# yuhang1008/WildGS-SLAM-Blackwell

Hardware: AMD Instinct MI355X
Metric: rasterised Gaussians/s fwd+bwd @1M pts 1080p; PSNR vs ref (higher is better)
Workload: dtype f32; 1 GPU; configs[2]: 1000000 Gaussians, 1920x1080, SH3, single-view fwd+bwd, pose grad on; gaussians=1000000, image=1920x1080, sh_degree=3, num_rendered=13015374, parallelism=dp1 (keyframe views), dp_exchange=none

## Files before the change

### wildgs-slam-blackwell_amd/csrc/capi.hip

```cpp
#include <cstdarg>
#include <cstdio>
#include <cstdlib>
#include <cstring>
#include <vector>

#include <immintrin.h>

#include "wgsr.h"
#include "wgsr_common.h"
#include "wgsr_internal.h"

namespace wgsr {

namespace {
thread_local char g_err[1024] = "";

struct HostCounters {
  uint32_t* buf = nullptr;
  hipEvent_t ev = nullptr;
  hipStream_t side = nullptr;
  hipEvent_t pre = nullptr;
  uint4* mbox = nullptr;
  uint32_t seq = 0;
};
// ... 109 lines not shown
        ms[r.stage] += t;
        count[r.stage] += 1;
      }
      pool.push_back(r.a);
      pool.push_back(r.b);
    }
    recs.clear();
  }
};
Prof g_prof;

struct StageTimer {
  Stage stage;
  hipStream_t s;
  hipEvent_t a = nullptr;
  StageTimer(Stage st, hipStream_t str) : stage(st), s(str) {
    if (((g_prof.mask >> st) & 1u) && (a = g_prof.get()) && hipEventRecord(a, s) != hipSuccess) a = nullptr;
  }
  ~StageTimer() {
    if (!a) return;
    hipEvent_t b = g_prof.get();
    if (b && hipEventRecord(b, s) == hipSuccess) g_prof.recs.push_back({stage, a, b});
    else g_prof.pool.push_back(a);
  }
};

struct Grid {
  int gx, gy, nt;
  explicit Grid(const wgsr_raster_args& a)
      : gx((a.W + kTile - 1) / kTile), gy((a.H + kTile - 1) / kTile), nt(gx * gy) {}
};

int sort_bits(int n) { return num_bits((uint32_t)n) > 0 ? num_bits((uint32_t)n) : 1; }

constexpr int kDefaultBinShift = 2;
constexpr int kSmallFrameTiles = 2048;
int bin_shift(const wgsr_raster_args& a) {
  const char* e = getenv("WGSR_BIN_SHIFT");
  const Grid g(a);
  int sh = e ? atoi(e) : (g.nt <= kSmallFrameTiles ? 1 : kDefaultBinShift);
  sh = sh < 0 ? 0 : (sh > kMaxBinShift ? kMaxBinShift : sh);
  return sh > 0 && g.nt > 65535 ? 0 : sh;
}
enum class DepthSched { kBins, kGlobal, kFull };
DepthSched depth_schedule(int bshift) {
  const char* e = getenv("WGSR_DEPTH_SORT");
  if (e && strcmp(e, "full") == 0) return DepthSched::kFull;
  if (!bshift || (e && strcmp(e, "global") == 0)) return DepthSched::kGlobal;
  return DepthSched::kBins;
}
size_t bin_depth_max_avg() {
  const char* e = getenv("WGSR_BIN_DEPTH_MAX_AVG");
  return e ? (size_t)strtoull(e, nullptr, 10) : (size_t)6144;
}
constexpr int kDepthBits = 32;
constexpr bool kFullDepthInAlt = ((kDepthBits + 7) / 8) % 2 == 1;
thread_local int64_t g_depth_order_off = -1;

int validate(const wgsr_raster_args* a) {
  if (!a) return set_error(WGSR_EINVAL, "null args");
  if (a->P < 0) return set_error(WGSR_EINVAL, "means3D must have dimensions (num_points, 3)");
  if (a->W <= 0 || a->H <= 0) return set_error(WGSR_EINVAL, "image size must be positive (got %dx%d)", a->W, a->H);
  if (a->P == 0) return WGSR_OK;
  if (!a->means3D || !a->opacities || !a->bg || !a->viewmatrix || !a->projmatrix || !a->campos)
    return set_error(WGSR_EINVAL, "missing required tensor");
  if ((a->shs == nullptr) == (a->colors == nullptr))
    return set_error(WGSR_EINVAL, "Please provide excatly one of either SHs or precomputed colors!");
  const bool sr = a->scales && a->rotations;
  if (sr == (a->cov3D_precomp != nullptr))
    return set_error(WGSR_EINVAL,
                     "Please provide exactly one of either scale/rotation pair or precomputed 3D covariance!");
  if (a->shs && (a->M <= 0 || a->D < 0 || a->D > 3 || (a->D + 1) * (a->D + 1) > a->M))
    return set_error(WGSR_EINVAL, "invalid SH configuration (degree %d, %d coefficients)", a->D, a->M);
  const Grid g(*a);
  if (g.gx > 65535 || g.gy > 65535) return set_error(WGSR_EINVAL, "image too large");
  return WGSR_OK;
}

#define HIPCHK(expr)                                                                          \
  do {                                                                                        \
    hipError_t _e = (expr);                                                                   \
    if (_e != hipSuccess) return set_error(WGSR_EHIP, "%s: %s", #expr, hipGetErrorString(_e)); \
  } while (0)

#define STAGE(a, s, expr)                   \
  do {                                      \
    HIPCHK(expr);                           \
    if ((a).debug) {                        \
      HIPCHK(hipStreamSynchronize(s));      \
      HIPCHK(hipGetLastError());            \
    }                                       \
  } while (0)

void* call_alloc(wgsr_alloc_fn fn, void* ctx, size_t bytes) { return fn ? fn(ctx, bytes) : nullptr; }

struct Fwd {
  const wgsr_raster_args& a;
  hipStream_t s;
  Grid grid; GeomLayout GL; ImageLayout IL;
  int bshift;
  float *out_color, *out_depth, *out_opacity;
  int32_t* n_touched;
  void *geom = nullptr, *image = nullptr;
  uint32_t* counter = nullptr;
  template <typename T> T* g(size_t off) const { return at<T>(geom, off); }
  template <typename T> T* im(size_t off) const { return at<T>(image, off); }
// ... 153 lines not shown
}

int queue_depth_fixup(const Fwd& f, HostCounters& hc, const Counts& c, const uint32_t** depth_order) {
  const GeomLayout& GL = f.GL;
  uint32_t hi = 0, nlo = 0;
  if (int e = read_depth_range(f, hc, c, &hi, &nlo)) return e;
  const DepthKeyPlan pl = depth_key_plan(hi, ~nlo);
  if (pl.extra_bits <= 0) return WGSR_OK;
  bool alt = false;
  { StageTimer T(kStDepthSort, f.s);
  STAGE(f.a, f.s, radix_sort_pairs(f.g<uint32_t>(GL.dkey_alt), f.g<uint32_t>(GL.dkey), f.g<uint32_t>(GL.dval_alt),
                                   f.g<uint32_t>(GL.dval), false, (size_t)f.a.P, pl.extra_shift, pl.R,
                                   f.g<uint32_t>(GL.hist), f.g<uint32_t>(GL.totals), f.s, &alt)); }
  *depth_order = f.g<uint32_t>(alt ? GL.dval : GL.dval_alt);
  return requeue_scan(f, *depth_order);
}

int queue_lists_and_render(const Fwd& f, void* binning, const BinningPlan& plan, const uint32_t* depth_order,
                           bool bin_depth, size_t NL, const uint32_t* ndev) {
  const wgsr_raster_args& a = f.a;
  hipStream_t s = f.s;
  const int bshift = f.bshift;
  const BinLayout& BL = plan.BL;
  uint32_t* lists = at<uint32_t>(binning, bshift ? BL.total : BL.point_g);
  uint2 *ranges = f.im<uint2>(f.IL.ranges), *tile_m = f.im<uint2>(f.IL.tile_m);
  uint32_t *tile_len = f.im<uint32_t>(f.IL.tile_len), *meta = f.im<uint32_t>(f.IL.meta);
  const uint32_t *sorted_keys = nullptr, *sorted_gid = nullptr;
  bool emit = false, bounds_done = false;
  if (NL > 0) {
    const int bits = sort_bits(bshift ? Bins(f.grid.gx, f.grid.gy, bshift).n : f.grid.nt);
    const bool odd = radix_passes(0, bits) % 2 == 1;
    uint32_t* vin = at<uint32_t>(binning, odd ? BL.slot_g : BL.point_g);
    uint32_t* valt = at<uint32_t>(binning, odd ? BL.point_g : BL.slot_g);
    size_t bs_off = 0;
    const size_t bs_words = bshift ? sort_sup_words(NL, 0, bits, &bs_off) : 0;
    ZeroJob zb{};
    zb.p[0] = reinterpret_cast<float*>(at<uint32_t>(binning, BL.hist) + bs_off);
    zb.n[0] = bs_words;
    zb.count = bs_words ? 1 : 0;
    { StageTimer T(kStDuplicate, s);
    if (bshift) {
      const uint32_t cap = ndev ? (uint32_t)NL : 0xFFFFFFFFu;
      STAGE(a, s, launch_duplicate_bins(a, f.geom, depth_order, bshift, at<uint8_t>(binning, BL.flag),
                                        at<uint32_t>(binning, BL.key), vin, true, zb, meta, s, cap, cap));
    } else {
      STAGE(a, s, launch_duplicate(a, f.geom, depth_order, (uint32_t)a.P, at<uint32_t>(binning, BL.key), vin,
                                   at<uint8_t>(binning, BL.flag), s));
    } }
    bool talt = false;
    uint2* bin_bounds = (bshift && (size_t)8 << bits <= (size_t)16 * f.grid.nt) ? tile_m : nullptr;
    { StageTimer T(kStTileSort, s);
    STAGE(a, s, radix_sort_pairs(at<uint32_t>(binning, BL.key), at<uint32_t>(binning, BL.key_alt), vin, valt, false,
                                 NL, 0, bits, at<uint32_t>(binning, BL.hist), at<uint32_t>(binning, BL.totals), s,
                                 &talt, bin_bounds, &bounds_done, bs_words != 0, ndev)); }
    if (talt != odd) return set_error(WGSR_EHIP, "internal: list sort parity");
    if (ndev && !bounds_done) return set_error(WGSR_EHIP, "internal: capacity mode without the sort's bin bounds");
    sorted_keys = at<uint32_t>(binning, talt ? BL.key_alt : BL.key);
    sorted_gid = at<uint32_t>(binning, BL.point_g);
    emit = bin_depth && bds_emit(bshift);
    if (bin_depth) {
      StageTimer T(kStTileSort, s);
      uint32_t* okeys = at<uint32_t>(binning, talt ? BL.key : BL.key_alt);
      uint32_t* ogid = at<uint32_t>(binning, BL.slot_g);
      STAGE(a, s, launch_bin_depth_sort(a, sorted_keys, sorted_gid, (uint32_t)NL, bshift, tile_m, bounds_done,
                                        at<uint32_t>(f.geom, f.GL.dkey), okeys, ogid,
                                        at<char>(binning, BL.total + plan.lists_bytes), s, emit ? lists : nullptr,
                                        ranges, tile_len, meta));
      bounds_done = true;
      if (!emit) {
        sorted_keys = okeys;
        sorted_gid = ogid;
      }
    }
  }
  { StageTimer T(kStRanges, s);
  if (emit) {
  } else if (bshift && NL > 0) {
    STAGE(a, s, launch_expand_bins(a, sorted_keys, sorted_gid, (uint32_t)NL, bshift, tile_m, bounds_done, lists,
                                   ranges, tile_len, meta, s));
  } else {
    STAGE(a, s, launch_ranges(sorted_keys, (uint32_t)NL, f.grid.nt, ranges, tile_len, meta, s));
  } }
  StageTimer T(kStRenderFwd, s);
  STAGE(a, s, launch_render_fwd(a, ranges, lists, f.geom, f.out_color, f.out_depth, f.out_opacity,
                                f.im<float>(f.IL.final_T), f.im<uint32_t>(f.IL.n_contrib), f.n_touched,
                                f.im<uint32_t>(f.IL.tile_m), s));
  return WGSR_OK;
}

}
}

using namespace wgsr;

extern "C" {

const char* wgsr_last_error(void) { return g_err; }

void wgsr_profile_enable(int on) {
  g_prof.flush();
  g_prof.mask = on == 1 ? ((1u << WGSR_NUM_STAGES) - 1u) : (on > 1 ? ((uint32_t)on >> 1) : 0u);
}

int wgsr_profile_read(double* ms, int64_t* counts, int n, int reset) {
  g_prof.flush();
  const int m = n < WGSR_NUM_STAGES ? n : WGSR_NUM_STAGES;
  for (int i = 0; i < m; ++i) {
// ... 333 lines not shown
```

### wildgs-slam-blackwell_amd/csrc/sort.hip

```cpp
#include <stdlib.h>
#include <string.h>

#include "wgsr_common.h"
#include "wgsr_internal.h"

namespace wgsr {

namespace {

__device__ __forceinline__ uint32_t block_excl_scan256(uint32_t v, uint32_t* s_tmp4, uint32_t* total) {
  const int t = threadIdx.x, w = t >> 6, lane = t & 63;
  uint32_t inc = wave_incl_scan(v);
  if (lane == 63) s_tmp4[w] = inc;
  __syncthreads();
  uint32_t base = 0, tot = 0;
#pragma unroll
  for (int i = 0; i < 4; ++i) {
    uint32_t x = s_tmp4[i];
    base += (i < w) ? x : 0u;
    tot += x;
  }
  __syncthreads();
  if (total) *total = tot;
  return base + inc - v;
}


template <int I>
__device__ __forceinline__ int load_run(const uint32_t* __restrict__ keys, size_t n, size_t e0, uint32_t (&k)[I]) {
  static_assert(I % 4 == 0, "load_run reads uint4s");
  if (e0 + I <= n) {
    const uint4* p = reinterpret_cast<const uint4*>(keys + e0);
#pragma unroll
    for (int q = 0; q < I / 4; ++q) {
      const uint4 v = p[q];
      k[4 * q] = v.x; k[4 * q + 1] = v.y; k[4 * q + 2] = v.z; k[4 * q + 3] = v.w;
    }
    return I;
  }
  const int nv = e0 < n ? (int)(n - e0) : 0;
#pragma unroll
  for (int j = 0; j < I; ++j) k[j] = j < nv ? keys[e0 + j] : 0u;
  return nv;
}

template <int I>
__device__ __forceinline__ void add_runs(uint32_t* h, const uint32_t (&k)[I], int nv, int shift, uint32_t mask) {
  if (nv <= 0) return;
  uint32_t cur = (k[0] >> shift) & mask, run = 0;
#pragma unroll
  for (int j = 0; j < I; ++j) {
    if (j < nv) {
      const uint32_t d = (k[j] >> shift) & mask;
      if (d != cur) {
        atomicAdd(&h[cur], run);
        cur = d;
        run = 0;
      }
      ++run;
    }
  }
  atomicAdd(&h[cur], run);
}

constexpr uint32_t kSupBlocks = kSortSupBlocks;
template <int I>
__global__ __launch_bounds__(256) void k_radix_hist(const uint32_t* __restrict__ keys, uint32_t n, int shift,
                                                    int bits, uint32_t nb, uint32_t* __restrict__ hist,
                                                    uint32_t* __restrict__ sup, uint32_t nsup,
                                                    const uint32_t* __restrict__ ndev) {
  __shared__ uint32_t s_h[256];
  const int t = threadIdx.x;
  if (ndev) n = min(n, *ndev);
  s_h[t] = 0;
  uint32_t k[I];
  const int nv = load_run<I>(keys, n, (size_t)blockIdx.x * (256 * I) + (size_t)t * I, k);
  __syncthreads();
  add_runs(s_h, k, nv, shift, (1u << bits) - 1u);
  __syncthreads();
  const uint32_t c = s_h[t];
  if (sup) {
    hist[(size_t)blockIdx.x * 256 + t] = c;
    if (c) atomicAdd(&sup[(size_t)(blockIdx.x / kSupBlocks) * 256 + t], c);
  } else {
// ... 86 lines not shown
  uint32_t gdig = 0;
  if (sup) {
    gdig = sup_digit_base(hist, sup, nb, nsup, bid, t, s_tmp, bounds, mask);
  } else {
    const uint32_t ex = block_excl_scan256(totals[t], s_tmp, nullptr);
    gdig = ex + hist[(size_t)t * nb + bid];
  }
#pragma unroll
  for (int j = 0; j < I; ++j) {
    const size_t e = base + (size_t)j * 64 + lane;
    const bool valid = e < n;
    const uint32_t d = (key[j] >> shift) & mask;
    const uint64_t peers = match_digit(d, bits, wave_ballot(valid));
    const int leader = __ffsll((unsigned long long)peers) - 1;
    uint32_t old = 0;
    if (valid && lane == leader) old = atomicAdd(&s_wcnt[w][d], (uint32_t)__popcll(peers));
    old = (uint32_t)__shfl((int)old, leader & 63, 64);
    rank[j] = old + lanes_below(peers);
  }
  __syncthreads();
  {
    const uint32_t c0 = s_wcnt[0][t], c1 = s_wcnt[1][t], c2 = s_wcnt[2][t], c3 = s_wcnt[3][t];
    const uint32_t cnt_d = c0 + c1 + c2 + c3;
    s_wcnt[0][t] = 0;
    s_wcnt[1][t] = c0;
    s_wcnt[2][t] = c0 + c1;
    s_wcnt[3][t] = c0 + c1 + c2;
    s_lbase[t] = block_excl_scan256(cnt_d, s_tmp, nullptr);
    s_gbase[t] = gdig;
  }
  __syncthreads();
#pragma unroll
  for (int j = 0; j < I; ++j) {
    const size_t e = base + (size_t)j * 64 + lane;
    const uint32_t d = (key[j] >> shift) & mask;
    const uint32_t slot = s_lbase[d] + s_wcnt[w][d] + rank[j];
    if (e < n) s_buf[slot] = make_uint2(key[j], val[j]);
  }
  __syncthreads();
  const uint32_t cnt = (size_t)n > blk0 ? (uint32_t)min((size_t)kTile, (size_t)n - blk0) : 0u;
#pragma unroll
  for (int r = 0; r < I; ++r) {
    const uint32_t i = (uint32_t)t + 256u * r;
    if (i < cnt) {
      const uint2 kv = s_buf[i];
      const uint32_t d = (kv.x >> shift) & mask;
      const uint32_t dst = s_gbase[d] + (i - s_lbase[d]);
      kout[dst] = kv.x;
      vout[dst] = kv.y;
    }
  }
}

template <int DIG, int I>
__global__ __launch_bounds__(256) void k_radix_hist_wide(const uint32_t* __restrict__ keys, uint32_t n, int shift,
                                                         int bits, uint32_t nb, uint32_t* __restrict__ hist,
                                                         const uint32_t* __restrict__ ndev) {
  __shared__ uint32_t s_h[DIG];
  const int t = threadIdx.x;
  if (ndev) n = min(n, *ndev);
#pragma unroll
  for (int k = 0; k < DIG / 256; ++k) s_h[t + 256 * k] = 0;
  uint32_t key[I];
  const int nv = load_run<I>(keys, n, (size_t)blockIdx.x * (256 * I) + (size_t)t * I, key);
  __syncthreads();
  add_runs(s_h, key, nv, shift, (1u << bits) - 1u);
  __syncthreads();
#pragma unroll
  for (int k = 0; k < DIG / 256; ++k) hist[(size_t)(t + 256 * k) * nb + blockIdx.x] = s_h[t + 256 * k];
}

template <int DIG, int I>
__global__ __launch_bounds__(256) void k_radix_scatter_wide(
    const uint32_t* __restrict__ kin, const uint32_t* __restrict__ vin, int iota, uint32_t n, int shift, int bits,
    uint32_t nb, const uint32_t* __restrict__ hist, const uint32_t* __restrict__ totals, uint32_t* __restrict__ kout,
    uint32_t* __restrict__ vout, uint2* __restrict__ digit_bounds, const uint32_t* __restrict__ ndev) {
  constexpr int kT = 256 * I, DPT = DIG / 256;
  if (ndev) {
    n = min(n, *ndev);
    if ((size_t)blockIdx.x * kT >= n && !(blockIdx.x == 0 && digit_bounds)) return;
  }
  __shared__ uint2 s_buf[kT];
  __shared__ uint32_t s_wcnt[4][DIG];
  __shared__ uint32_t s_lbase[DIG];
  __shared__ uint32_t s_gbase[DIG];
  __shared__ uint32_t s_tmp[4];
  const int t = threadIdx.x, w = t >> 6, lane = t & 63;
  const uint32_t mask = (1u << bits) - 1u;
#pragma unroll
  for (int i = 0; i < 4 * DPT; ++i) (&s_wcnt[0][0])[t + 256 * i] = 0;
  const uint32_t bid = blockIdx.x;
  const size_t blk0 = (size_t)bid * kT;
  const size_t base = blk0 + (size_t)w * (64 * I);
  uint32_t key[I], val[I], rank[I];
#pragma unroll
  for (int j = 0; j < I; ++j) {
    const size_t e = base + (size_t)j * 64 + lane;
    const bool valid = e < n;
    key[j] = valid ? kin[e] : 0u;
    val[j] = iota ? (uint32_t)e : (valid ? vin[e] : 0u);
  }
  {
    uint32_t tot[DPT], s = 0;
#pragma unroll
    for (int k = 0; k < DPT; ++k) { tot[k] = totals[t * DPT + k]; s += tot[k]; }
    uint32_t run = block_excl_scan256(s, s_tmp, nullptr);
#pragma unroll
    for (int k = 0; k < DPT; ++k) {
      const int d = t * DPT + k;
      s_gbase[d] = run + hist[(size_t)d * nb + bid];
      if (digit_bounds && bid == 0) digit_bounds[d] = make_uint2(run, run + tot[k]);
      run += tot[k];
    }
  }
#pragma unroll
  for (int j = 0; j < I; ++j) {
    const size_t e = base + (size_t)j * 64 + lane;
    const bool valid = e < n;
    const uint32_t d = (key[j] >> shift) & mask;
    const uint64_t peers = match_digit(d, bits, wave_ballot(valid));
    const int leader = __ffsll((unsigned long long)peers) - 1;
    uint32_t old = 0;
    if (valid && lane == leader) old = atomicAdd(&s_wcnt[w][d], (uint32_t)__popcll(peers));
    old = (uint32_t)__shfl((int)old, leader & 63, 64);
    rank[j] = old + lanes_below(peers);
  }
  __syncthreads();
  {
    uint32_t cnt[DPT], s = 0;
#pragma unroll
    for (int k = 0; k < DPT; ++k) {
      const int d = t * DPT + k;
      const uint32_t c0 = s_wcnt[0][d], c1 = s_wcnt[1][d], c2 = s_wcnt[2][d], c3 = s_wcnt[3][d];
      cnt[k] = c0 + c1 + c2 + c3;
      s += cnt[k];
      s_wcnt[0][d] = 0;
      s_wcnt[1][d] = c0;
      s_wcnt[2][d] = c0 + c1;
      s_wcnt[3][d] = c0 + c1 + c2;
    }
    uint32_t run = block_excl_scan256(s, s_tmp, nullptr);
#pragma unroll
    for (int k = 0; k < DPT; ++k) {
      s_lbase[t * DPT + k] = run;
      run += cnt[k];
    }
  }
  __syncthreads();
#pragma unroll
  for (int j = 0; j < I; ++j) {
    const size_t e = base + (size_t)j * 64 + lane;
    const uint32_t d = (key[j] >> shift) & mask;
    const uint32_t slot = s_lbase[d] + s_wcnt[w][d] + rank[j];
    if (e < n) s_buf[slot] = make_uint2(key[j], val[j]);
  }
  __syncthreads();
  const uint32_t cnt = (size_t)n > blk0 ? (uint32_t)min((size_t)kT, (size_t)n - blk0) : 0u;
#pragma unroll
  for (int r = 0; r < I; ++r) {
    const uint32_t i = (uint32_t)t + 256u * r;
    if (i < cnt) {
      const uint2 kv = s_buf[i];
      const uint32_t d = (kv.x >> shift) & mask;
      const uint32_t dst = s_gbase[d] + (i - s_lbase[d]);
      kout[dst] = kv.x;
      vout[dst] = kv.y;
    }
  }
}

static_assert(kRectPairLanes == 64, "one range word per lane");
__device__ __forceinline__ int bitlen32(uint32_t x) {
  return x ? 32 - __clz((int)x) : 0;
}
__device__ __forceinline__ uint32_t wave_max_u32_uniform(uint32_t x) {
  x = max(x, (uint32_t)__builtin_amdgcn_update_dpp(0, (int)x, 0xB1, 0xf, 0xf, true));
  x = max(x, (uint32_t)__builtin_amdgcn_update_dpp(0, (int)x, 0x4E, 0xf, 0xf, true));
  x = max(x, (uint32_t)__builtin_amdgcn_update_dpp(0, (int)x, 0x114, 0xf, 0xf, true));
  x = max(x, (uint32_t)__builtin_amdgcn_update_dpp(0, (int)x, 0x118, 0xf, 0xf, true));
  const uint32_t a = (uint32_t)__builtin_amdgcn_readlane((int)x, 15), b = (uint32_t)__builtin_amdgcn_readlane((int)x, 31);
  const uint32_t c = (uint32_t)__builtin_amdgcn_readlane((int)x, 47), d = (uint32_t)__builtin_amdgcn_readlane((int)x, 63);
  return max(max(a, b), max(c, d));
}
__device__ __forceinline__ uint2 depth_range_reduce(const uint32_t* __restrict__ range) {
  const int lane = threadIdx.x & 63;
  return make_uint2(wave_max_u32_uniform(range[lane]), wave_max_u32_uniform(range[kRectPairLanes + lane]));
}
__device__ __forceinline__ DepthKeyPlan depth_plan_from2(const uint32_t* __restrict__ range2) {
  return depth_key_plan(range2[0], ~range2[1]);
}

template <int I, int PASS>
__global__ __launch_bounds__(256) void k_depth_hist(const uint32_t* __restrict__ keys, uint32_t n,
                                                    const uint32_t* __restrict__ range, uint32_t* __restrict__ range2,
                                                    uint32_t* __restrict__ hist, uint32_t* __restrict__ sup) {
  __shared__ uint32_t s_h[kDepthMaxDigits];
  const int t = threadIdx.x;
  uint32_t k[I];
  const int nv = load_run<I>(keys, n, (size_t)blockIdx.x * (256 * I) + (size_t)t * I, k);
#pragma unroll
  for (int q = 0; q < kDepthMaxDigits / 256; ++q) s_h[t + 256 * q] = 0;
  DepthKeyPlan pl;
  if (PASS == 0) {
    const uint2 r = depth_range_reduce(range);
    if (blockIdx.x == 0 && t == 0) {
      range2[0] = r.x;
      range2[1] = r.y;
    }
    pl = depth_key_plan(r.x, ~r.y);
  } else {
    pl = depth_plan_from2(range2);
  }
  const int shift = pl.shift[PASS], bits = pl.bits[PASS];
// ... 269 lines not shown
  const uint32_t b0 = min(nbs, t * per), b1 = min(nbs, b0 + per);
  uint2 acc = make_uint2(0u, 0u);
  for (uint32_t b = b0; b < b1; b += 8) {
    uint2 v[8];
#pragma unroll
    for (int u = 0; u < 8; ++u) v[u] = b + u < b1 ? bsum[b + u] : make_uint2(0u, 0u);
#pragma unroll
    for (int u = 0; u < 8; ++u) { acc.x += v[u].x; acc.y += v[u].y; }
  }
  const uint32_t ia = wave_incl_scan(acc.x), ib = wave_incl_scan(acc.y);
  if (lane == 63) s_w[w] = make_uint2(ia, ib);
  __syncthreads();
  uint2 run = make_uint2(ia - acc.x, ib - acc.y), tot = make_uint2(0u, 0u);
#pragma unroll
  for (int k = 0; k < NW; ++k) {
    const uint2 x = s_w[k];
    if (k < w) { run.x += x.x; run.y += x.y; }
    tot.x += x.x;
    tot.y += x.y;
  }
  for (uint32_t b = b0; b < b1; b += 8) {
    uint2 v[8];
#pragma unroll
    for (int u = 0; u < 8; ++u) v[u] = b + u < b1 ? bsum[b + u] : make_uint2(0u, 0u);
#pragma unroll
    for (int u = 0; u < 8; ++u) {
      if (b + u < b1) bsum[b + u] = run;
      run.x += v[u].x;
      run.y += v[u].y;
    }
  }
  if (t == 0) bsum[nbs] = tot;
}

}

static bool wide_pass(int bits) { return bits > 8 && bits <= 10; }

int radix_passes(int begin_bit, int end_bit) {
  const int bits = end_bit - begin_bit;
  if (bits <= 0) return 0;
  return wide_pass(bits) ? 1 : (bits + 7) / 8;
}

size_t sort_sup_words(size_t n, int begin_bit, int end_bit, size_t* offset_words) {
  const int bits = end_bit - begin_bit;
  if (offset_words) *offset_words = 0;
  if (n == 0 || bits <= 0 || wide_pass(bits)) return 0;
  const uint32_t nb = sort_blocks(n);
  if (offset_words) *offset_words = 256 * (size_t)nb;
  return 256 * (size_t)((nb + kSupBlocks - 1) / kSupBlocks) * ((bits + 7) / 8);
}

template <int I>
static hipError_t radix_sort_tiled(uint32_t* keys, uint32_t* keys_alt, uint32_t* vals, uint32_t* vals_alt,
                                   bool vals_iota, size_t n, int begin_bit, int end_bit, uint32_t* status,
                                   uint32_t* totals, hipStream_t stream, bool* result_in_alt, uint2* digit_bounds,
                                   bool* bounds_done, bool sup_zeroed, const uint32_t* ndev) {
  const uint32_t nb = sort_blocks(n);
  if (wide_pass(end_bit - begin_bit) && n <= (size_t)kStCount) {
    const int bits = end_bit - begin_bit;
    if (bits <= 9) {
      hipLaunchKernelGGL((k_radix_hist_wide<512, I>), dim3(nb), dim3(256), 0, stream, keys, (uint32_t)n, begin_bit,
                         bits, nb, status, ndev);
      hipLaunchKernelGGL(k_radix_rowscan, dim3(512), dim3(256), 0, stream, status, nb, totals);
      hipLaunchKernelGGL((k_radix_scatter_wide<512, I>), dim3(nb), dim3(256), 0, stream, keys, vals,
                         vals_iota ? 1 : 0, (uint32_t)n, begin_bit, bits, nb, status, totals, keys_alt, vals_alt,
                         begin_bit == 0 ? digit_bounds : nullptr, ndev);
    } else {
      hipLaunchKernelGGL((k_radix_hist_wide<1024, I>), dim3(nb), dim3(256), 0, stream, keys, (uint32_t)n, begin_bit,
                         bits, nb, status, ndev);
      hipLaunchKernelGGL(k_radix_rowscan, dim3(1024), dim3(256), 0, stream, status, nb, totals);
      hipLaunchKernelGGL((k_radix_scatter_wide<1024, I>), dim3(nb), dim3(256), 0, stream, keys, vals,
                         vals_iota ? 1 : 0, (uint32_t)n, begin_bit, bits, nb, status, totals, keys_alt, vals_alt,
                         begin_bit == 0 ? digit_bounds : nullptr, ndev);
    }
    *result_in_alt = true;
    if (bounds_done) *bounds_done = digit_bounds && begin_bit == 0;
    return hipGetLastError();
  }
  const int passes = (end_bit - begin_bit + 7) / 8;
  if (passes > kMaxSortPasses || n > (size_t)kStCount) return hipErrorInvalidValue;
  uint32_t* ghist = totals;
  const uint32_t nsup = (nb + kSupBlocks - 1) / kSupBlocks;
  uint32_t* sup = status + 256 * (size_t)nb;
  if (!sup_zeroed) {
    hipError_t e = hipMemsetAsync(sup, 0, 4 * 256 * (size_t)nsup * passes, stream);
    if (e != hipSuccess) return e;
  }
  uint32_t *ki = keys, *ko = keys_alt, *vi = vals, *vo = vals_alt;
  bool iota = vals_iota;
  const int per = (end_bit - begin_bit + passes - 1) / passes;
  for (int p = 0; p < passes; ++p) {
    const int shift = begin_bit + per * p;
    const int bits = min(per, end_bit - shift);
    uint32_t* sp = sup + (size_t)p * 256 * nsup;
    hipLaunchKernelGGL(k_radix_hist<I>, dim3(nb), dim3(256), 0, stream, ki, (uint32_t)n, shift, bits, nb, status,
                       sp, nsup, ndev);
    uint2* db = (passes == 1 && begin_bit == 0) ? digit_bounds : nullptr;
    hipLaunchKernelGGL(k_radix_scatter<I>, dim3(nb), dim3(256), 0, stream, ki, vi, iota ? 1 : 0, (uint32_t)n, shift,
                       bits, nb, status, ghist, ko, vo, sp, nsup, db, ndev);
    if (db && bounds_done) *bounds_done = true;
    iota = false;
    uint32_t* tk = ki; ki = ko; ko = tk;
    uint32_t* tv = vi; vi = vo; vo = tv;
    *result_in_alt = !*result_in_alt;
  }
  return hipGetLastError();
}

hipError_t radix_sort_pairs(uint32_t* keys, uint32_t* keys_alt, uint32_t* vals, uint32_t* vals_alt, bool vals_iota,
                            size_t n, int begin_bit, int end_bit, uint32_t* status, uint32_t* totals,
                            hipStream_t stream, bool* result_in_alt, uint2* digit_bounds, bool* bounds_done,
                            bool sup_zeroed, const uint32_t* ndev) {
  *result_in_alt = false;
  if (bounds_done) *bounds_done = false;
  if (n == 0 || end_bit <= begin_bit) {
    if (vals_iota && n > 0) {
      return hipErrorInvalidValue;
    }
    return hipSuccess;
  }
  switch (sort_items(n)) {
    case kTinySortItems:
      return radix_sort_tiled<kTinySortItems>(keys, keys_alt, vals, vals_alt, vals_iota, n, begin_bit, end_bit, status,
                                              totals, stream, result_in_alt, digit_bounds, bounds_done, sup_zeroed,
                                              ndev);
    case kSmallSortItems:
      return radix_sort_tiled<kSmallSortItems>(keys, keys_alt, vals, vals_alt, vals_iota, n, begin_bit, end_bit,
                                               status, totals, stream, result_in_alt, digit_bounds, bounds_done,
                                               sup_zeroed, ndev);
    default:
      return radix_sort_tiled<kSortItems>(keys, keys_alt, vals, vals_alt, vals_iota, n, begin_bit, end_bit, status,
                                          totals, stream, result_in_alt, digit_bounds, bounds_done, sup_zeroed,
                                          ndev);
  }
}

template <int I>
static hipError_t depth_sort_tiled(uint32_t* keys, uint32_t* keys_alt, uint32_t* vals, uint32_t* vals_alt, size_t n,
                                   const uint32_t* range, uint32_t* range2, uint32_t* scratch, hipStream_t s) {
  const uint32_t nb = (uint32_t)((n + 256 * I - 1) / (256 * I)), nsup = (nb + kSupBlocks - 1) / kSupBlocks;
  uint32_t* hist = scratch;
  uint32_t* sup = scratch + depth_sort_sup_offset_words(n);
  const size_t sup_pass = (size_t)kDepthMaxDigits * nsup;
  const uint32_t un = (uint32_t)n;
  hipLaunchKernelGGL((k_depth_hist<I, 0>), dim3(nb), dim3(256), 0, s, keys, un, range, range2, hist, sup);
  hipLaunchKernelGGL((k_depth_scatter<I, 0>), dim3(nb), dim3(256), 0, s, keys, vals, un, range2, hist, sup, nsup,
                     keys_alt, vals_alt);
  hipLaunchKernelGGL((k_depth_hist<I, 1>), dim3(nb), dim3(256), 0, s, keys_alt, un, range, range2, hist,
                     sup + sup_pass);
  hipLaunchKernelGGL((k_depth_scatter<I, 1>), dim3(nb), dim3(256), 0, s, keys_alt, vals_alt, un, range2, hist,
                     sup + sup_pass, nsup, keys, vals);
  hipLaunchKernelGGL((k_depth_hist<I, 2>), dim3(nb), dim3(256), 0, s, keys, un, range, range2, hist,
                     sup + 2 * sup_pass);
  hipLaunchKernelGGL((k_depth_scatter<I, 2>), dim3(nb), dim3(256), 0, s, keys, vals, un, range2, hist,
                     sup + 2 * sup_pass, nsup, keys_alt, vals_alt);
  return hipGetLastError();
}

hipError_t launch_depth_sort(uint32_t* keys, uint32_t* keys_alt, uint32_t* vals, uint32_t* vals_alt, size_t n,
                             const uint32_t* range, uint32_t* range2, uint32_t* scratch, hipStream_t s) {
  if (n == 0) return hipSuccess;
  if (n > (size_t)kStCount) return hipErrorInvalidValue;
  switch (sort_items(n)) {
    case kTinySortItems:
      return depth_sort_tiled<kTinySortItems>(keys, keys_alt, vals, vals_alt, n, range, range2, scratch, s);
    case kSmallSortItems:
      return depth_sort_tiled<kSmallSortItems>(keys, keys_alt, vals, vals_alt, n, range, range2, scratch, s);
    default:
      return depth_sort_tiled<kSortItems>(keys, keys_alt, vals, vals_alt, n, range, range2, scratch, s);
  }
}

hipError_t exclusive_scan_gather(const uint32_t* vals, const uint32_t* idx, size_t n, uint32_t* out,
                                 uint32_t* scatter_out, uint32_t* bsum, uint32_t* total_out, hipStream_t stream,
                                 uint32_t stride) {
  const uint32_t nbs = (uint32_t)((n + kScanTile - 1) / kScanTile);
  if (n == 0) {
    hipError_t e = hipMemsetAsync(out, 0, sizeof(uint32_t), stream);
    if (e == hipSuccess && total_out) e = hipMemsetAsync(total_out, 0, sizeof(uint32_t), stream);
    return e;
  }
  hipLaunchKernelGGL(k_scan_reduce, dim3(nbs), dim3(256), 0, stream, vals, stride, idx, (uint32_t)n, bsum);
  hipLaunchKernelGGL(k_scan_bsum, dim3(1), dim3(256), 0, stream, bsum, nbs, total_out);
  hipLaunchKernelGGL(k_scan_down, dim3(nbs), dim3(256), 0, stream, vals, stride, idx, (uint32_t)n, bsum, out,
                     scatter_out);
  return hipGetLastError();
// ... 15 lines not shown
```

### wildgs-slam-blackwell_amd/csrc/wgsr_common.h

```cpp
#pragma once

#include <hip/hip_runtime.h>
#include <stdint.h>

namespace wgsr {

constexpr int kTile = 16;
constexpr int kTilePix = kTile * kTile;
constexpr int kWave = 64;
constexpr float kNearZ = 0.2f;
constexpr float kMinAlpha = 1.0f / 255.0f;
constexpr float kMaxAlpha = 0.99f;
constexpr float kMinT = 0.0001f;
constexpr float kL2E = 1.4426950408889634f;
constexpr float kConicSq = -0.5f * kL2E;
constexpr float kConicXY = -kL2E;
constexpr float kUnConicSq = -2.0f / kL2E, kUnConicXY = -1.0f / kL2E;

typedef float v2f __attribute__((ext_vector_type(2)));

__device__ __forceinline__ int lane_id() { return __lane_id(); }

__device__ __forceinline__ uint32_t lanes_below(uint64_t mask) {
  return __builtin_amdgcn_mbcnt_hi((uint32_t)(mask >> 32),
// ... 510 lines not shown
#pragma unroll
  for (int r = 0; r < 3; ++r)
#pragma unroll
    for (int k = 0; k < 3; ++k) c.Rw[r][k] = c.view[4 * k + r];
  c.W = W; c.H = H; c.tanx = tanx; c.tany = tany;
  c.fx = W / (2.0f * tanx);
  c.fy = H / (2.0f * tany);
}

__device__ __forceinline__ void ewa_T(const Cam& c, f3 t, float T[2][3], f3& tc, float& xmul, float& ymul) {
#pragma clang fp contract(off)
  const float limx = 1.3f * c.tanx, limy = 1.3f * c.tany;
  const float txtz = t.x / t.z, tytz = t.y / t.z;
  tc = {fminf(limx, fmaxf(-limx, txtz)) * t.z, fminf(limy, fmaxf(-limy, tytz)) * t.z, t.z};
  xmul = (txtz < -limx || txtz > limx) ? 0.f : 1.f;
  ymul = (tytz < -limy || tytz > limy) ? 0.f : 1.f;
  const float J00 = c.fx / tc.z, J02 = -(c.fx * tc.x) / (tc.z * tc.z);
  const float J11 = c.fy / tc.z, J12 = -(c.fy * tc.y) / (tc.z * tc.z);
#pragma unroll
  for (int k = 0; k < 3; ++k) {
    T[0][k] = J00 * c.Rw[0][k] + J02 * c.Rw[2][k];
    T[1][k] = J11 * c.Rw[1][k] + J12 * c.Rw[2][k];
  }
}

__device__ __forceinline__ void sym3(const float c6[6], float S[3][3]) {
  S[0][0] = c6[0]; S[0][1] = c6[1]; S[0][2] = c6[2];
  S[1][0] = c6[1]; S[1][1] = c6[3]; S[1][2] = c6[4];
  S[2][0] = c6[2]; S[2][1] = c6[4]; S[2][2] = c6[5];
}

__device__ __forceinline__ void cov2d(const float T[2][3], const float S[3][3], float& a, float& b, float& c) {
#pragma clang fp contract(off)
  float ST0[3], ST1[3];
#pragma unroll
  for (int i = 0; i < 3; ++i) {
    ST0[i] = S[i][0] * T[0][0] + S[i][1] * T[0][1] + S[i][2] * T[0][2];
    ST1[i] = S[i][0] * T[1][0] + S[i][1] * T[1][1] + S[i][2] * T[1][2];
  }
  a = T[0][0] * ST0[0] + T[0][1] * ST0[1] + T[0][2] * ST0[2] + 0.3f;
  b = T[0][0] * ST1[0] + T[0][1] * ST1[1] + T[0][2] * ST1[2];
  c = T[1][0] * ST1[0] + T[1][1] * ST1[1] + T[1][2] * ST1[2] + 0.3f;
}

__host__ __device__ constexpr size_t align256(size_t x) { return (x + 255) & ~size_t(255); }

#ifndef WGSR_SMALL_SORT_ITEMS
#define WGSR_SMALL_SORT_ITEMS 8
#endif
#ifndef WGSR_TINY_SORT_ITEMS
#define WGSR_TINY_SORT_ITEMS 4
#endif
constexpr int kSortItems = 16;
constexpr int kSmallSortItems = WGSR_SMALL_SORT_ITEMS;
constexpr int kTinySortItems = WGSR_TINY_SORT_ITEMS;
constexpr size_t kSmallSortN = size_t(1) << 21;
constexpr size_t kTinySortN = size_t(1) << 18;
constexpr int kScanTile = 1024;
constexpr int kPackedScanTile = 256;

__host__ __device__ inline int sort_items(size_t n) {
  return n <= kTinySortN ? kTinySortItems : (n <= kSmallSortN ? kSmallSortItems : kSortItems);
}
__host__ __device__ inline uint32_t sort_blocks(size_t n) {
  const size_t tile = 256 * (size_t)sort_items(n);
  return (uint32_t)((n + tile - 1) / tile);
}
constexpr int kRectPairLanes = 64;
constexpr size_t kDepthRangeOffset = 16 + 3 * 8 * kRectPairLanes;
constexpr size_t kCounterBytes = kDepthRangeOffset + 2 * 4 * kRectPairLanes;

struct PublishJob {
  const uint32_t* counter = nullptr;
  uint4* host = nullptr;
  uint32_t seq = 0;
};
__device__ __forceinline__ void publish_counts(const PublishJob& pj, int lane) {
  const unsigned long long* partial = reinterpret_cast<const unsigned long long*>(pj.counter + 4);
  unsigned long long v[3];
#pragma unroll
  for (int k = 0; k < 3; ++k) {
    v[k] = partial[k * kRectPairLanes + lane];
#pragma unroll
    for (int off = 32; off >= 1; off >>= 1) v[k] += (unsigned long long)__shfl_xor((long long)v[k], off, 64);
  }
  if (lane == 0) {
    const bool big = ((v[0] | v[1] | v[2]) >> 32) != 0;
    *pj.host = make_uint4((pj.seq << 8) | (pj.counter[1] & 0x7Fu) | (big ? 0x80u : 0u), (uint32_t)v[0],
                          (uint32_t)v[1], (uint32_t)v[2]);
  }
}
static_assert(kRectPairLanes == 64, "publish_counts: one lane per partial");

constexpr int kDepthPasses = 3;
constexpr int kDepthMaxDigitBits = 10;
constexpr int kDepthMaxDigits = 1 << kDepthMaxDigitBits;
struct DepthKeyPlan {
  uint32_t lo_r, cul;
  int R;
  int shift[kDepthPasses], bits[kDepthPasses];
  int extra_shift, extra_bits;
};
__host__ __device__ inline DepthKeyPlan depth_key_plan(uint32_t hi, uint32_t lo) {
  DepthKeyPlan p;
  if (hi < lo) {
    p.lo_r = 0u;
// ... 142 lines not shown
```

### wildgs-slam-blackwell_amd/csrc/wgsr_internal.h

```cpp
#pragma once

#include <hip/hip_runtime.h>
#include <stdint.h>

#include "wgsr.h"

namespace wgsr {

int radix_passes(int begin_bit, int end_bit);
hipError_t radix_sort_pairs(uint32_t* keys, uint32_t* keys_alt, uint32_t* vals, uint32_t* vals_alt, bool vals_iota,
                            size_t n, int begin_bit, int end_bit, uint32_t* status, uint32_t* totals,
                            hipStream_t stream, bool* result_in_alt,
                            uint2* digit_bounds = nullptr, bool* bounds_done = nullptr, bool sup_zeroed = false,
                            const uint32_t* ndev = nullptr);
size_t sort_sup_words(size_t n, int begin_bit, int end_bit, size_t* offset_words);

hipError_t launch_depth_sort(uint32_t* keys, uint32_t* keys_alt, uint32_t* vals, uint32_t* vals_alt, size_t n,
                             const uint32_t* range, uint32_t* range2, uint32_t* scratch, hipStream_t s);

hipError_t exclusive_scan_gather(const uint32_t* vals, const uint32_t* idx, size_t n, uint32_t* out,
                                 uint32_t* scatter_out, uint32_t* bsum, uint32_t* total_out, hipStream_t stream,
                                 uint32_t stride = 1);

hipError_t packed_scan_blocks(const uint32_t* packed, uint32_t stride, const uint32_t* idx, size_t n, void* bsum,
                              hipStream_t stream,
                              void* bsup = nullptr, const PublishJob& pub = PublishJob{});

int num_bits(uint32_t n);

int set_error(int code, const char* fmt, ...);

struct RasterGrid {
  int gx, gy, ntiles;
};

hipError_t launch_preprocess(const wgsr_raster_args& a, void* geom, int32_t* radii, int32_t* n_touched,
                             uint32_t* err_flag, unsigned long long* rect_pairs, int bshift, const ZeroJob& zero, hipStream_t s, uint32_t* meta);
hipError_t launch_cap_counts(const unsigned long long* partial, uint64_t cap_rect, uint64_t cap_bin, uint32_t* counts,
                             uint32_t* meta, hipStream_t s);
hipError_t launch_duplicate_bins(const wgsr_raster_args& a, void* geom, const uint32_t* depth_order, int bshift,
                                 uint8_t* pflag, uint32_t* keys, uint32_t* vals, bool bsup, const ZeroJob& zero,
                                 uint32_t* meta, hipStream_t s, uint32_t cap_slots = 0xFFFFFFFFu,
                                 uint32_t cap_pairs = 0xFFFFFFFFu);
hipError_t launch_duplicate(const wgsr_raster_args& a, const void* geom, const uint32_t* sorted_g, uint32_t P,
                            uint32_t* keys, uint32_t* slot_g, uint8_t* pflag, hipStream_t s);
uint32_t argsort_small_max();
hipError_t launch_argsort_small(const uint32_t* keys, uint32_t n, uint32_t* perm, hipStream_t s);
hipError_t launch_bin_depth_sort(const wgsr_raster_args& a, const uint32_t* sorted_keys, const uint32_t* sorted_g,
                                 uint32_t NB, int bshift, uint2* bounds, bool bounds_done, const uint32_t* gdepth,
                                 uint32_t* okeys, uint32_t* ogid, void* scratch, hipStream_t s,
                                 uint32_t* lists = nullptr, uint2* ranges = nullptr, uint32_t* tile_len = nullptr,
                                 uint32_t* meta = nullptr);
hipError_t launch_expand_bins(const wgsr_raster_args& a, const uint32_t* sorted_keys, const uint32_t* sorted_g,
                              uint32_t NB, int bshift, uint2* bounds, bool bounds_done, uint32_t* lists, uint2* ranges,
                              uint32_t* tile_len, uint32_t* meta, hipStream_t s);
hipError_t launch_ranges(const uint32_t* sorted_keys, uint32_t N, int ntiles, uint2* ranges, uint32_t* len,
                         uint32_t* meta, hipStream_t s);
hipError_t launch_tile_order(const uint32_t* work_quads, int ntiles, uint32_t* order, hipStream_t s);
hipError_t launch_render_fwd(const wgsr_raster_args& a, const uint2* ranges, const uint32_t* point_g,
                             const void* geom, float* out_color, float* out_depth,
                             float* out_opacity, float* final_T, uint32_t* n_contrib, int32_t* n_touched,
                             uint32_t* tile_m4, hipStream_t s);
hipError_t launch_zero_u32(uint32_t* p, size_t n, hipStream_t s);
hipError_t launch_check_tile_lists(const wgsr_raster_args& a, int bshift, uint64_t num_rendered, const void* binning,
                                   const void* image, uint32_t* bad, hipStream_t s);
hipError_t launch_mark_visible(int P, const float* means3D, const float* view, const float* proj, uint8_t* present,
                               hipStream_t s);
// ... 24 lines not shown
```

Baseline: 1.433 billion Gaussians/s.

## Template wide radix pass on block size and add LDS match-table ranking

The single-pass wide radix sort kernels (histogram and scatter) now take the thread count as a template parameter. With the default item count they run 512 threads per block, each handling fewer keys, and per-wave counters and scans are generalised to any number of waves. For the default item count the scatter kernel also replaces the ballot-based digit peer matching with an LDS table of 64-bit masks built by atomicOr, reusing the staging buffer. The aim is more parallelism per tile and a cheaper match step for 9-10 bit digits, at the cost of more LDS atomics and per-thread bookkeeping.

Measured after the change: 1.448 billion Gaussians/s (median of 6 runs). 1.1% higher.

```diff
diff --git a/wildgs-slam-blackwell_amd/csrc/capi.hip b/wildgs-slam-blackwell_amd/csrc/capi.hip
--- a/wildgs-slam-blackwell_amd/csrc/capi.hip
+++ b/wildgs-slam-blackwell_amd/csrc/capi.hip
@@ -185,6 +185,10 @@
 size_t bin_depth_max_avg() {
   const char* e = getenv("WGSR_BIN_DEPTH_MAX_AVG");
   return e ? (size_t)strtoull(e, nullptr, 10) : (size_t)6144;
+}
+int bin_sort_threads() {
+  const char* e = getenv("WGSR_BIN_SORT_THREADS");
+  return e ? atoi(e) : 0;
 }
 constexpr int kDepthBits = 32;
 constexpr bool kFullDepthInAlt = ((kDepthBits + 7) / 8) % 2 == 1;
@@ -444,7 +448,8 @@
     { StageTimer T(kStTileSort, s);
     STAGE(a, s, radix_sort_pairs(at<uint32_t>(binning, BL.key), at<uint32_t>(binning, BL.key_alt), vin, valt, false,
                                  NL, 0, bits, at<uint32_t>(binning, BL.hist), at<uint32_t>(binning, BL.totals), s,
-                                 &talt, bin_bounds, &bounds_done, bs_words != 0, ndev)); }
+                                 &talt, bin_bounds, &bounds_done, bs_words != 0, ndev,
+                                 bshift ? bin_sort_threads() : 0)); }
     if (talt != odd) return set_error(WGSR_EHIP, "internal: list sort parity");
     if (ndev && !bounds_done) return set_error(WGSR_EHIP, "internal: capacity mode without the sort's bin bounds");
     sorted_keys = at<uint32_t>(binning, talt ? BL.key_alt : BL.key);
diff --git a/wildgs-slam-blackwell_amd/csrc/sort.hip b/wildgs-slam-blackwell_amd/csrc/sort.hip
--- a/wildgs-slam-blackwell_amd/csrc/sort.hip
+++ b/wildgs-slam-blackwell_amd/csrc/sort.hip
@@ -25,11 +25,23 @@
   return base + inc - v;
 }
 
+template <int NW>
+__device__ __forceinline__ uint32_t block_excl_scan_waves(uint32_t v, uint32_t* s_tmp) {
+  const int t = threadIdx.x, w = t >> 6, lane = t & 63;
+  uint32_t inc = wave_incl_scan(v);
+  if (lane == 63) s_tmp[w] = inc;
+  __syncthreads();
+  uint32_t base = 0;
+#pragma unroll
+  for (int i = 0; i < NW; ++i) base += (i < w) ? s_tmp[i] : 0u;
+  __syncthreads();
+  return base + inc - v;
+}
+
 
 template <int I>
 __device__ __forceinline__ int load_run(const uint32_t* __restrict__ keys, size_t n, size_t e0, uint32_t (&k)[I]) {
-  static_assert(I % 4 == 0, "load_run reads uint4s");
-  if (e0 + I <= n) {
+  if (I % 4 == 0 && e0 + I <= n) {
     const uint4* p = reinterpret_cast<const uint4*>(keys + e0);
 #pragma unroll
     for (int q = 0; q < I / 4; ++q) {
@@ -222,49 +234,54 @@
   }
 }
 
-template <int DIG, int I>
-__global__ __launch_bounds__(256) void k_radix_hist_wide(const uint32_t* __restrict__ keys, uint32_t n, int shift,
-                                                         int bits, uint32_t nb, uint32_t* __restrict__ hist,
-                                                         const uint32_t* __restrict__ ndev) {
+template <int DIG, int NT, int I>
+__global__ __launch_bounds__(NT) void k_radix_hist_wide(const uint32_t* __restrict__ keys, uint32_t n, int shift,
+                                                        int bits, uint32_t nb, uint32_t* __restrict__ hist,
+                                                        const uint32_t* __restrict__ ndev) {
+  constexpr int kT = 256 * I, K = kT / NT;
+  static_assert(K >= 1 && K * NT == kT, "whole keys per thread");
   __shared__ uint32_t s_h[DIG];
   const int t = threadIdx.x;
   if (ndev) n = min(n, *ndev);
-#pragma unroll
-  for (int k = 0; k < DIG / 256; ++k) s_h[t + 256 * k] = 0;
-  uint32_t key[I];
-  const int nv = load_run<I>(keys, n, (size_t)blockIdx.x * (256 * I) + (size_t)t * I, key);
+  for (int d = t; d < DIG; d += NT) s_h[d] = 0;
+  uint32_t key[K];
+  const int nv = load_run<K>(keys, n, (size_t)blockIdx.x * kT + (size_t)t * K, key);
   __syncthreads();
   add_runs(s_h, key, nv, shift, (1u << bits) - 1u);
   __syncthreads();
-#pragma unroll
-  for (int k = 0; k < DIG / 256; ++k) hist[(size_t)(t + 256 * k) * nb + blockIdx.x] = s_h[t + 256 * k];
-}
-
-template <int DIG, int I>
-__global__ __launch_bounds__(256) void k_radix_scatter_wide(
+  for (int d = t; d < DIG; d += NT) hist[(size_t)d * nb + blockIdx.x] = s_h[d];
+}
+
+template <int DIG, int NT, int I>
+__global__ __launch_bounds__(NT) void k_radix_scatter_wide(
     const uint32_t* __restrict__ kin, const uint32_t* __restrict__ vin, int iota, uint32_t n, int shift, int bits,
     uint32_t nb, const uint32_t* __restrict__ hist, const uint32_t* __restrict__ totals, uint32_t* __restrict__ kout,
     uint32_t* __restrict__ vout, uint2* __restrict__ digit_bounds, const uint32_t* __restrict__ ndev) {
-  constexpr int kT = 256 * I, DPT = DIG / 256;
+  constexpr int kT = 256 * I, K = kT / NT, NW = NT / 64, DPT = DIG >= NT ? DIG / NT : 1;
+  static_assert(K >= 1 && K * NT == kT && NW * 64 == NT, "whole keys per thread, whole waves");
   if (ndev) {
     n = min(n, *ndev);
     if ((size_t)blockIdx.x * kT >= n && !(blockIdx.x == 0 && digit_bounds)) return;
   }
   __shared__ uint2 s_buf[kT];
-  __shared__ uint32_t s_wcnt[4][DIG];
+  __shared__ uint32_t s_wcnt[NW][DIG];
   __shared__ uint32_t s_lbase[DIG];
   __shared__ uint32_t s_gbase[DIG];
-  __shared__ uint32_t s_tmp[4];
+  __shared__ uint32_t s_tmp[NW];
   const int t = threadIdx.x, w = t >> 6, lane = t & 63;
   const uint32_t mask = (1u << bits) - 1u;
-#pragma unroll
-  for (int i = 0; i < 4 * DPT; ++i) (&s_wcnt[0][0])[t + 256 * i] = 0;
+  const bool own = t * DPT < DIG;
+  for (int i = t; i < NW * DIG; i += NT) (&s_wcnt[0][0])[i] = 0;
+  constexpr bool kTable = I == kSortItems && NW * DIG <= kT;
+  unsigned long long* s_match = reinterpret_cast<unsigned long long*>(s_buf);
+  if (kTable)
+    for (int i = t; i < NW * DIG; i += NT) s_match[i] = 0ull;
   const uint32_t bid = blockIdx.x;
   const size_t blk0 = (size_t)bid * kT;
-  const size_t base = blk0 + (size_t)w * (64 * I);
-  uint32_t key[I], val[I], rank[I];
-#pragma unroll
-  for (int j = 0; j < I; ++j) {
+  const size_t base = blk0 + (size_t)w * (64 * K);
+  uint32_t key[K], val[K], rank[K];
+#pragma unroll
+  for (int j = 0; j < K; ++j) {
     const size_t e = base + (size_t)j * 64 + lane;
     const bool valid = e < n;
     key[j] = valid ? kin[e] : 0u;
@@ -273,22 +290,32 @@
   {
     uint32_t tot[DPT], s = 0;
 #pragma unroll
-    for (int k = 0; k < DPT; ++k) { tot[k] = totals[t * DPT + k]; s += tot[k]; }
-    uint32_t run = block_excl_scan256(s, s_tmp, nullptr);
+    for (int k = 0; k < DPT; ++k) { tot[k] = own ? totals[t * DPT + k] : 0u; s += tot[k]; }
+    uint32_t run = block_excl_scan_waves<NW>(s, s_tmp);
 #pragma unroll
     for (int k = 0; k < DPT; ++k) {
       const int d = t * DPT + k;
-      s_gbase[d] = run + hist[(size_t)d * nb + bid];
-      if (digit_bounds && bid == 0) digit_bounds[d] = make_uint2(run, run + tot[k]);
+      if (own) {
+        s_gbase[d] = run + hist[(size_t)d * nb + bid];
+        if (digit_bounds && bid == 0) digit_bounds[d] = make_uint2(run, run + tot[k]);
+      }
       run += tot[k];
     }
   }
 #pragma unroll
-  for (int j = 0; j < I; ++j) {
+  for (int j = 0; j < K; ++j) {
     const size_t e = base + (size_t)j * 64 + lane;
     const bool valid = e < n;
     const uint32_t d = (key[j] >> shift) & mask;
-    const uint64_t peers = match_digit(d, bits, wave_ballot(valid));
+    uint64_t peers;
+    if (kTable) {
+      unsigned long long* m = &s_match[w * DIG + d];
+      if (valid) atomicOr(m, 1ull << lane);
+      peers = valid ? *m : 0ull;
+      if (valid) *m = 0ull;
+    } else {
+      peers = match_digit(d, bits, wave_ballot(valid));
+    }
     const int leader = __ffsll((unsigned long long)peers) - 1;
     uint32_t old = 0;
     if (valid && lane == leader) old = atomicAdd(&s_wcnt[w][d], (uint32_t)__popcll(peers));
@@ -301,24 +328,28 @@
 #pragma unroll
     for (int k = 0; k < DPT; ++k) {
       const int d = t * DPT + k;
-      const uint32_t c0 = s_wcnt[0][d], c1 = s_wcnt[1][d], c2 = s_wcnt[2][d], c3 = s_wcnt[3][d];
-      cnt[k] = c0 + c1 + c2 + c3;
-      s += cnt[k];
-      s_wcnt[0][d] = 0;
-      s_wcnt[1][d] = c0;
-      s_wcnt[2][d] = c0 + c1;
-      s_wcnt[3][d] = c0 + c1 + c2;
-    }
-    uint32_t run = block_excl_scan256(s, s_tmp, nullptr);
+      uint32_t run = 0;
+      if (own) {
+#pragma unroll
+        for (int q = 0; q < NW; ++q) {
+          const uint32_t c = s_wcnt[q][d];
+          s_wcnt[q][d] = run;
+          run += c;
+        }
+      }
+      cnt[k] = run;
+      s += run;
+    }
+    uint32_t run = block_excl_scan_waves<NW>(s, s_tmp);
 #pragma unroll
     for (int k = 0; k < DPT; ++k) {
-      s_lbase[t * DPT + k] = run;
+      if (own) s_lbase[t * DPT + k] = run;
       run += cnt[k];
     }
   }
   __syncthreads();
 #pragma unroll
-  for (int j = 0; j < I; ++j) {
+  for (int j = 0; j < K; ++j) {
     const size_t e = base + (size_t)j * 64 + lane;
     const uint32_t d = (key[j] >> shift) & mask;
     const uint32_t slot = s_lbase[d] + s_wcnt[w][d] + rank[j];
@@ -327,8 +358,8 @@
   __syncthreads();
   const uint32_t cnt = (size_t)n > blk0 ? (uint32_t)min((size_t)kT, (size_t)n - blk0) : 0u;
 #pragma unroll
-  for (int r = 0; r < I; ++r) {
-    const uint32_t i = (uint32_t)t + 256u * r;
+  for (int r = 0; r < K; ++r) {
+    const uint32_t i = (uint32_t)t + (uint32_t)NT * r;
     if (i < cnt) {
       const uint2 kv = s_buf[i];
       const uint32_t d = (kv.x >> shift) & mask;
@@ -704,29 +735,37 @@
   return 256 * (size_t)((nb + kSupBlocks - 1) / kSupBlocks) * ((bits + 7) / 8);
 }
 
+template <int DIG, int NT, int I>
+static void launch_wide_pass(uint32_t* keys, uint32_t* keys_alt, uint32_t* vals, uint32_t* vals_alt, bool vals_iota,
+                             uint32_t n, int begin_bit, int bits, uint32_t nb, uint32_t* status, uint32_t* totals,
+                             hipStream_t stream, uint2* digit_bounds, const uint32_t* ndev) {
+  hipLaunchKernelGGL((k_radix_hist_wide<DIG, NT, I>), dim3(nb), dim3(NT), 0, stream, keys, n, begin_bit, bits, nb,
+                     status, ndev);
+  hipLaunchKernelGGL(k_radix_rowscan, dim3(DIG), dim3(256), 0, stream, status, nb, totals);
+  hipLaunchKernelGGL((k_radix_scatter_wide<DIG, NT, I>), dim3(nb), dim3(NT), 0, stream, keys, vals, vals_iota ? 1 : 0,
+                     n, begin_bit, bits, nb, status, totals, keys_alt, vals_alt, digit_bounds, ndev);
+}
+
 template <int I>
 static hipError_t radix_sort_tiled(uint32_t* keys, uint32_t* keys_alt, uint32_t* vals, uint32_t* vals_alt,
                                    bool vals_iota, size_t n, int begin_bit, int end_bit, uint32_t* status,
                                    uint32_t* totals, hipStream_t stream, bool* result_in_alt, uint2* digit_bounds,
-                                   bool* bounds_done, bool sup_zeroed, const uint32_t* ndev) {
+                                   bool* bounds_done, bool sup_zeroed, const uint32_t* ndev, int wide_threads) {
   const uint32_t nb = sort_blocks(n);
   if (wide_pass(end_bit - begin_bit) && n <= (size_t)kStCount) {
     const int bits = end_bit - begin_bit;
+    int nt = wide_threads;
+    if (nt != 256 && nt != 512 && nt != 1024) nt = I == kSortItems ? kWideSortThreads : 256;
+    uint2* db = begin_bit == 0 ? digit_bounds : nullptr;
+#define WGSR_WIDE(DIG, NT)                                                                                         \
+  launch_wide_pass<DIG, NT, I>(keys, keys_alt, vals, vals_alt, vals_iota, (uint32_t)n, begin_bit, bits, nb, status, \
+                               totals, stream, db, ndev)
     if (bits <= 9) {
-      hipLaunchKernelGGL((k_radix_hist_wide<512, I>), dim3(nb), dim3(256), 0, stream, keys, (uint32_t)n, begin_bit,
-                         bits, nb, status, ndev);
-      hipLaunchKernelGGL(k_radix_rowscan, dim3(512), dim3(256), 0, stream, status, nb, totals);
-      hipLaunchKernelGGL((k_radix_scatter_wide<512, I>), dim3(nb), dim3(256), 0, stream, keys, vals,
-                         vals_iota ? 1 : 0, (uint32_t)n, begin_bit, bits, nb, status, totals, keys_alt, vals_alt,
-                         begin_bit == 0 ? digit_bounds : nullptr, ndev);
+      if (nt == 256) WGSR_WIDE(512, 256); else if (nt == 512) WGSR_WIDE(512, 512); else WGSR_WIDE(512, 1024);
     } else {
-      hipLaunchKernelGGL((k_radix_hist_wide<1024, I>), dim3(nb), dim3(256), 0, stream, keys, (uint32_t)n, begin_bit,
-                         bits, nb, status, ndev);
-      hipLaunchKernelGGL(k_radix_rowscan, dim3(1024), dim3(256), 0, stream, status, nb, totals);
-      hipLaunchKernelGGL((k_radix_scatter_wide<1024, I>), dim3(nb), dim3(256), 0, stream, keys, vals,
-                         vals_iota ? 1 : 0, (uint32_t)n, begin_bit, bits, nb, status, totals, keys_alt, vals_alt,
-                         begin_bit == 0 ? digit_bounds : nullptr, ndev);
-    }
+      if (nt == 256) WGSR_WIDE(1024, 256); else if (nt == 512) WGSR_WIDE(1024, 512); else WGSR_WIDE(1024, 1024);
+    }
+#undef WGSR_WIDE
     *result_in_alt = true;
     if (bounds_done) *bounds_done = digit_bounds && begin_bit == 0;
     return hipGetLastError();
@@ -764,7 +803,7 @@
 hipError_t radix_sort_pairs(uint32_t* keys, uint32_t* keys_alt, uint32_t* vals, uint32_t* vals_alt, bool vals_iota,
                             size_t n, int begin_bit, int end_bit, uint32_t* status, uint32_t* totals,
                             hipStream_t stream, bool* result_in_alt, uint2* digit_bounds, bool* bounds_done,
-                            bool sup_zeroed, const uint32_t* ndev) {
+                            bool sup_zeroed, const uint32_t* ndev, int wide_threads) {
   *result_in_alt = false;
   if (bounds_done) *bounds_done = false;
   if (n == 0 || end_bit <= begin_bit) {
@@ -777,15 +816,15 @@
     case kTinySortItems:
       return radix_sort_tiled<kTinySortItems>(keys, keys_alt, vals, vals_alt, vals_iota, n, begin_bit, end_bit, status,
                                               totals, stream, result_in_alt, digit_bounds, bounds_done, sup_zeroed,
-                                              ndev);
+                                              ndev, wide_threads);
     case kSmallSortItems:
       return radix_sort_tiled<kSmallSortItems>(keys, keys_alt, vals, vals_alt, vals_iota, n, begin_bit, end_bit,
                                                status, totals, stream, result_in_alt, digit_bounds, bounds_done,
-                                               sup_zeroed, ndev);
+                                               sup_zeroed, ndev, wide_threads);
     default:
       return radix_sort_tiled<kSortItems>(keys, keys_alt, vals, vals_alt, vals_iota, n, begin_bit, end_bit, status,
                                           totals, stream, result_in_alt, digit_bounds, bounds_done, sup_zeroed,
-                                          ndev);
+                                          ndev, wide_threads);
   }
 }
 
diff --git a/wildgs-slam-blackwell_amd/csrc/wgsr_common.h b/wildgs-slam-blackwell_amd/csrc/wgsr_common.h
--- a/wildgs-slam-blackwell_amd/csrc/wgsr_common.h
+++ b/wildgs-slam-blackwell_amd/csrc/wgsr_common.h
@@ -586,6 +586,7 @@
 #define WGSR_TINY_SORT_ITEMS 4
 #endif
 constexpr int kSortItems = 16;
+constexpr int kWideSortThreads = 512;
 constexpr int kSmallSortItems = WGSR_SMALL_SORT_ITEMS;
 constexpr int kTinySortItems = WGSR_TINY_SORT_ITEMS;
 constexpr size_t kSmallSortN = size_t(1) << 21;
diff --git a/wildgs-slam-blackwell_amd/csrc/wgsr_internal.h b/wildgs-slam-blackwell_amd/csrc/wgsr_internal.h
--- a/wildgs-slam-blackwell_amd/csrc/wgsr_internal.h
+++ b/wildgs-slam-blackwell_amd/csrc/wgsr_internal.h
@@ -12,7 +12,7 @@
                             size_t n, int begin_bit, int end_bit, uint32_t* status, uint32_t* totals,
                             hipStream_t stream, bool* result_in_alt,
                             uint2* digit_bounds = nullptr, bool* bounds_done = nullptr, bool sup_zeroed = false,
-                            const uint32_t* ndev = nullptr);
+                            const uint32_t* ndev = nullptr, int wide_threads = 0);
 size_t sort_sup_words(size_t n, int begin_bit, int end_bit, size_t* offset_words);
 
 hipError_t launch_depth_sort(uint32_t* keys, uint32_t* keys_alt, uint32_t* vals, uint32_t* vals_alt, size_t n,
```
